# templeblock/audioSignalProcess

Hardware: AMD Instinct MI355X
Metric: audio frames/sec (10 ms @16 kHz) Wiener NS (higher is better)
Workload: dtype f32

## Files before the change

audiosignalprocess_amd/csrc/ns_kernels1.hip:

```cpp
#include <hip/hip_runtime.h>

#include "handoff.h"
#include "ns_device.h"
#include "ns_layout.h"
#include "ns_pair_fft.h"

namespace {
using namespace asphandoff;
using namespace aspns_dev;
using namespace aspns_pair;

__device__ __forceinline__ unsigned long long ns_cu_tag() {
  const unsigned hw = __builtin_amdgcn_s_getreg((7 << 11) | (8 << 6) | 4);
  const unsigned xcc = __builtin_amdgcn_s_getreg((3 << 11) | (0 << 6) | 20);
  return (unsigned long long)((xcc << 8) | hw);
}

constexpr int NS3 = 3;

__device__ __forceinline__ int ns_cold(int x) {
  asm volatile("" : "+v"(x));
  return x;
}
template <typename P>
__device__ __forceinline__ const P* ns_cold(const P* p) {
  asm volatile("" : "+s"(p));
  return p;
}

struct NsFlowArgs {
  HandoffArgs hand;
  unsigned want;
  int slot0;
  int ring;
  unsigned per;
  unsigned steps;
  unsigned walk;
};

template <bool IO16>
__device__ __forceinline__ float4 load_frame4(const float* in, size_t idx) {
  if constexpr (IO16) {
    const short4 a = *reinterpret_cast<const short4*>(reinterpret_cast<const short*>(in) + idx);
    return make_float4((float)a.x, (float)a.y, (float)a.z, (float)a.w);
  } else {
    return *reinterpret_cast<const float4*>(in + idx);
  }
}

constexpr int kImgDwords = aspns::kOffVec + aspns::V_HOT_COUNT * aspns::kVecStride;
constexpr int kImgVec4 = kImgDwords / (64 * 4);
static_assert(kImgDwords == 1792 && kImgDwords % (64 * 4) == 0, "the image is copied as whole 16-byte pieces per lane");
typedef __attribute__((address_space(3))) float lds_f32;
typedef __attribute__((address_space(3))) f32x2v lds_f32x2;
typedef __attribute__((address_space(3))) f32x4v lds_f32x4;

template <bool FLOW>
struct StateAcc {
  float* st;
  __amdgpu_buffer_rsrc_t rs;
  lds_f32* img;
  __device__ __forceinline__ StateAcc(float* p, float* image) : st(p), img((lds_f32*)image) {
    if constexpr (FLOW) rs = __builtin_amdgcn_make_buffer_rsrc(p, 0, aspns::kStreamDwords * 4, 0x00020000);
  }
  __device__ __forceinline__ float ld1(int uni, int vec) const {
    if constexpr (FLOW) return uni < kImgDwords ? img[uni + vec] : sc1_load1(rs, vec * 4, uni * 4);
    else return st[uni + vec];
  }
  __device__ __forceinline__ float2 ld2(int uni, int vec) const {
    if constexpr (FLOW) {
      if (uni >= kImgDwords) return sc1_load2(rs, vec * 4, uni * 4);
      const f32x2v v = *reinterpret_cast<const lds_f32x2*>(img + uni + vec);
      return make_float2(v.x, v.y);
    } else {
      return *reinterpret_cast<const float2*>(st + uni + vec);
    }
  }
  __device__ __forceinline__ float4 ld4(int uni, int vec) const {
    if constexpr (FLOW) {
      if (uni >= kImgDwords) return sc1_load4(rs, vec * 4, uni * 4);
      const f32x4v v = *reinterpret_cast<const lds_f32x4*>(img + uni + vec);
      return make_float4(v.x, v.y, v.z, v.w);
    } else {
      return *reinterpret_cast<const float4*>(st + uni + vec);
    }
  }
  __device__ __forceinline__ void st1(int uni, int vec, float v) const {
    if constexpr (FLOW) {
      if (uni < kImgDwords) img[uni + vec] = v;
      else sc1_store1(rs, vec * 4, uni * 4, v);
    } else {
      st[uni + vec] = v;
    }
  }
  __device__ __forceinline__ void st2(int uni, int vec, float a, float b) const {
    if constexpr (FLOW) {
      if (uni < kImgDwords) *reinterpret_cast<lds_f32x2*>(img + uni + vec) = f32x2v{a, b};
      else sc1_store2(rs, vec * 4, uni * 4, a, b);
    } else {
      *reinterpret_cast<float2*>(st + uni + vec) = make_float2(a, b);
    }
  }
  __device__ __forceinline__ void st4(int uni, int vec, float4 x) const {
    if constexpr (FLOW) {
      if (uni < kImgDwords) *reinterpret_cast<lds_f32x4*>(img + uni + vec) = f32x4v{x.x, x.y, x.z, x.w};
      else sc1_store4(rs, vec * 4, uni * 4, x);
    } else {
      *reinterpret_cast<float4*>(st + uni + vec) = x;
    }
  }
  __device__ __forceinline__ void image_request(int lane, float4 (&v)[kImgVec4]) const {
#pragma unroll
    for (int i = 0; i < kImgVec4; ++i) v[i] = sc1_load4(rs, lane * 16, i * 1024);
  }
  __device__ __forceinline__ void image_fill(int lane, const float4 (&v)[kImgVec4]) const {
#pragma unroll
    for (int i = 0; i < kImgVec4; ++i)
      *reinterpret_cast<lds_f32x4*>(img + i * 256 + 4 * lane) = f32x4v{v[i].x, v[i].y, v[i].z, v[i].w};
  }
  __device__ __forceinline__ void image_write_back(int lane) const {
#pragma unroll
    for (int i = 0; i < kImgVec4; ++i) {
      const f32x4v v = *reinterpret_cast<const lds_f32x4*>(img + i * 256 + 4 * lane);
      sc1_store4(rs, lane * 16, i * 1024, make_float4(v.x, v.y, v.z, v.w));
    }
  }
};

template <bool IO16, bool FLOW>
__global__ __launch_bounds__(256, 4) void ns_frame1_kernel(float* __restrict__ state,
                                                           int32_t* __restrict__ hist_all,
                                                           const NsTables* __restrict__ T,
                                                           const float* __restrict__ in,
                                                           float* __restrict__ out,
                                                           int num_streams,
                                                           unsigned long long* __restrict__ stamps,
                                                           int stamp_mode, NsFlowArgs fa) {
#ifdef NS1_BUDGET
#define NS_STAMP(k)                                                                \
  __builtin_amdgcn_sched_barrier(0);                                               \
  asm volatile("; NS_PHASE " #k);                                                  \
  __builtin_amdgcn_sched_barrier(0);
#define NS_STEADY(x) __builtin_assume(x)
#else
  const int stamp_on = (stamps != nullptr && threadIdx.x < 64) ? (stamp_mode != 0 ? 1 : 2) : 0;
#define NS_STAMP(k)                                                                          \
  if (__builtin_amdgcn_readfirstlane(stamp_on) != 0 && threadIdx.x == 0) {                   \
    __builtin_amdgcn_sched_barrier(0);                                                       \
    if (stamp_on == 1) {                                                                     \
      if ((k) == 0 || (k) == 1 || (k) == 14 || (k) == 15)                                    \
        stamps[blockIdx.x * 4 + ((k) == 0 ? 0 : (k) == 1 ? 1 : (k) == 14 ? 2 : 3)] =        \
            __builtin_amdgcn_s_memrealtime() | ((k) == 0 ? ns_cu_tag() << 48 : 0ull);       \
    } else if (FLOW ? (blockIdx.x == gridDim.x / 2 && flow_j == fa.steps / 2)                \
                    : blockIdx.x == 0) {                                                     \
      stamps[k] = __builtin_amdgcn_s_memtime();                                              \
    }                                                                                        \
    __builtin_amdgcn_sched_barrier(0);                                                       \
  }
#define NS_STEADY(x)
#endif
  unsigned flow_j = 0, flow_end = 1, flow_slot = 0;
  if constexpr (FLOW) {
    flow_j = blockIdx.y * fa.walk;
    flow_end = flow_j + fa.walk < fa.steps ? flow_j + fa.walk : fa.steps;
    flow_slot = ((unsigned)fa.slot0 + flow_j) % (unsigned)fa.ring;
  } else {
    NS_STAMP(0)
  }
  __shared__ __align__(16) float2 lds[4][130];
  __shared__ __align__(16) float tabs[3 * 64 * 4 + 32 * 4 * 2];
  __shared__ __align__(16) float wins[kAnal];
  __shared__ __align__(16) double exp2s[64];
  __shared__ __align__(16) double2 logts[128];
  __shared__ __align__(16) float imgs[FLOW ? 4 : 1][FLOW ? kImgDwords : 4];
  const int tid = threadIdx.x;
  const float4* tab_src = tid < 192 ? reinterpret_cast<const float4*>(&T->tw[0][0][0]) + tid
                                    : reinterpret_cast<const float4*>(&T->spl[0][0][0]) + (tid - 192);
  const float4 tab_v = *tab_src;
  const float4 win_v = reinterpret_cast<const float4*>(T->window)[tid & 63];
  const double exp2_v = T->exp2_64[tid & 63];
  const double2 logt_v = reinterpret_cast<const double2*>(T->logtab)[tid & 127];
  const int lane = tid & 63;
  const int diagbits = T->diag[lane];
  const int wv = __builtin_amdgcn_readfirstlane(tid >> 6);
  float2* tile = lds[wv];
  const int lam = lane >> 1, h = lane & 1;
  const int g = lam >> 4, q = lam & 15;
  const int binA = q + 64 * g + 16 * h;
  const uint32_t gmask = g ? 0x80000000u : 0u;
  const int stream_raw = blockIdx.x * 4 + wv;
  bool wave_live = stream_raw < num_streams;
  const int stream = wave_live ? stream_raw : num_streams - 1;
  float* __restrict__ st = state + (size_t)stream * kStreamDwords;
  int32_t* __restrict__ hist = hist_all + (size_t)stream * kHistDwords;
  const StateAcc<FLOW> sa(st, FLOW ? imgs[wv] : nullptr);
  float* outj = out;

  float sv;
#define SC_I(k) __builtin_amdgcn_readlane(__float_as_int(sv), (k))
#define SC_F(k) __int_as_float(SC_I(k))
#define SC_SET_I(k, val) sv = writelane_bits<(k)>(sv, (int)(val))
#define SC_SET_F(k, val) sv = setlane_vgpr<(k)>(sv, (val))
  float4 s4;
  float2 carryA, carryB;
  float4 s4in = make_float4(0.f, 0.f, 0.f, 0.f);
  const size_t frame_uni = (size_t)stream * kBlockL;
  auto flow_load_in = [&](unsigned slot) __attribute__((always_inline)) {
    const int lane_c = ns_cold(lane);
    const unsigned frame_lane = 4u * (unsigned)((lane_c < 24 ? 24 : lane_c) - 24);
    const float* base = IO16 ? reinterpret_cast<const float*>(reinterpret_cast<const short*>(in + (size_t)slot * fa.per) + frame_uni)
                             : in + (size_t)slot * fa.per + frame_uni;
    s4in = load_frame4<IO16>(base, frame_lane);
  };
  auto flow_head = [&]() __attribute__((always_inline)) {
    NS_STAMP(0)
    outj = out + (size_t)flow_slot * fa.per;
    const int lane_c = ns_cold(lane);
    const float4 ha = sa.ld4(kOffAnaHist, 4 * (lane_c < 24 ? lane_c : 23));
    const bool hsel = lane_c < 24;
    s4.x = hsel ? ha.x : s4in.x;
    s4.y = hsel ? ha.y : s4in.y;
    s4.z = hsel ? ha.z : s4in.z;
    s4.w = hsel ? ha.w : s4in.w;
    const int q2_c = lane_c & 30;
    carryA = sa.ld2(kOffSynt, q2_c + 32 * (lane_c & 1));
    carryB = sa.ld2(kOffSynt, q2_c + 64);
  };
  [[maybe_unused]] float4 img_v[FLOW ? kImgVec4 : 1];
  if constexpr (FLOW) {
    flow_load_in(flow_slot);
    if (wave_live) wave_live = handoff_wait(fa.hand, fa.want + flow_j, stream, lane);
    if (wave_live) sa.image_request(lane, img_v);
  } else {
    sv = st[kOffScalars + lane];
    float* hbuf = st + kOffAnaHist;
    if (!IO16) {
      const float* src = lane < 24 ? hbuf + 4 * lane : in + (size_t)stream * kBlockL + 4 * (lane - 24);
      s4 = *reinterpret_cast<const float4*>(src);
    } else {
      const int lh = lane < 24 ? lane : 23, li = lane < 24 ? 24 : lane;
      const float4 ha = *reinterpret_cast<const float4*>(hbuf + 4 * lh);
      const short* in16 = reinterpret_cast<const short*>(in) + (size_t)stream * kBlockL + 4 * (li - 24);
      const short4 a = *reinterpret_cast<const short4*>(in16);
      const bool hsel = lane < 24;
      s4.x = hsel ? ha.x : (float)a.x;
      s4.y = hsel ? ha.y : (float)a.y;
      s4.z = hsel ? ha.z : (float)a.z;
      s4.w = hsel ? ha.w : (float)a.w;
    }
    carryA = *reinterpret_cast<const float2*>(st + kOffSynt + 2 * q + 32 * h);
    carryB = *reinterpret_cast<const float2*>(st + kOffSynt + 2 * q + 64);
  }

  reinterpret_cast<float4*>(tabs)[tid] = tab_v;
  if (tid < 64) exp2s[tid] = exp2_v;
  if (tid < 128) logts[tid] = logt_v;
  if (tid >= 192) reinterpret_cast<float4*>(wins)[tid - 192] = win_v;
  if constexpr (FLOW) {
    if (wave_live) sa.image_fill(lane, img_v);
  }
  __syncthreads();
  if (!wave_live) return;
  if constexpr (FLOW) {
    sv = sa.ld1(kOffScalars, lane);
    flow_head();
  }
  const float* tws = tabs;
  const float* spls = tabs + 3 * 64 * 4;
  const PairFftLane fl = pair_fft_lane(lane, diagbits);

#define LOADV(dst, f)                                                                          \
  {                                                                                            \
    const float2 v2_ = sa.ld2(kOffVec + (f)*kVecStride, 2 * lane);                             \
    dst[0] = v2_.x; dst[1] = v2_.y;                                                            \
  }
#define LOADT(dst, f) dst[2] = SC_F(S_TAIL0 + (f));
#define LOAD3(dst, f) LOADV(dst, f) LOADT(dst, f)
#define STORE3(f, srcv)                                                                        \
  {                                                                                            \
    sa.st2(kOffVec + (f)*kVecStride, 2 * lane, srcv[0], srcv[1]);                              \
    SC_SET_F(S_TAIL0 + (f), srcv[2]);                                                          \
  }
#define NS_NEXT_FRAME()                                                                        \
  if constexpr (FLOW) {                                                                        \
    flow_slot = flow_slot + 1u == (unsigned)fa.ring ? 0u : flow_slot + 1u;                     \
    if (flow_j + 1u < flow_end) flow_load_in(flow_slot);                                       \
  }
#define NS_STREAM_DONE()                                                                       \
  if constexpr (FLOW) {                                                                        \
    const bool walk_done_ = flow_j + 1u >= flow_end;                                           \
    if (walk_done_) {                                                                          \
      const int lane_w_ = ns_cold(lane);                                                       \
      sa.st1(kOffScalars, lane_w_, sv);                                                        \
      lds_sync1();                                                                             \
      sa.image_write_back(lane_w_);                                                            \
      handoff_drain();                                                                         \
    }                                                                                          \
    NS_STAMP(16)                                                                               \
    if (walk_done_) {                                                                          \
      if (lane == 0) handoff_publish(fa.hand.seq + stream, fa.want + flow_j);                  \
      return;                                                                                  \
    }                                                                                          \
    ++flow_j;                                                                                  \
    lds_sync1();                                                                               \
    flow_head();                                                                               \
    continue;                                                                                  \
  } else {                                                                                     \
    return;                                                                                    \
  }

  for (;;) {
    float LQ[3][NS3], DEN[3][NS3], quant[NS3];
    float smooth[NS3], noisePrev[NS3], magnPrevA[NS3], logLrt[NS3], avgPause[NS3];


    const float4 w4 = *reinterpret_cast<const float4*>(wins + 4 * lane);
    const float wx0 = w4.x * s4.x, wx1 = w4.y * s4.y, wx2 = w4.z * s4.z, wx3 = w4.w * s4.w;
    float epart = wx0 * wx0;
    epart += wx1 * wx1;
    epart += wx2 * wx2;
    epart += wx3 * wx3;
    const float energy1 = wave_sum_bcast(epart);

    {
      const int lane_c = ns_cold(lane);
      if (lane_c >= 40) sa.st4(kOffAnaHist, 4 * (lane_c - 40), s4);
    }

    NS_STEADY(energy1 != 0.0f);
    if (energy1 == 0.0f) {
      float* y = IO16 ? reinterpret_cast<float*>(reinterpret_cast<short*>(outj) + (size_t)stream * kBlockL)
                      : outj + (size_t)stream * kBlockL;
      NS_NEXT_FRAME()
      const int lane_c = ns_cold(lane);
      float2 o01 = make_float2(0.f, 0.f);
      if (lane_c < 48) o01 = sa.ld2(kOffSynt, 2 * lane_c);
      __builtin_amdgcn_fence(__ATOMIC_ACQ_REL, "wavefront");
      store2p<IO16>(y, 2 * lane_c, sat16p(o01.x), sat16p(o01.y));
      if (lane_c < 16) store2p<IO16>(y, 128 + 2 * lane_c, 0.f, 0.f);
      if (lane_c < 48) sa.st2(kOffSynt, 2 * lane_c, 0.f, 0.f);
      NS_STREAM_DONE()
    }

    LOADV(LQ[0], V_LQ0) LOADV(LQ[1], V_LQ1) LOADV(LQ[2], V_LQ2)
    LOADV(DEN[0], V_DEN0) LOADV(DEN[1], V_DEN1) LOADV(DEN[2], V_DEN2)
    LOADV(quant, V_QUANT)
    LOADT(quant, V_QUANT)
    NS_STAMP(1)
    *reinterpret_cast<float4*>(&tile[2 * lane]) = make_float4(wx0, wx1, wx2, wx3);
    lds_sync1();
    f32x2 er, ei;
    {
      f32x2 ea, eb;
      cft128_passes1(tile, tws, fl, lane, ea, eb);
      radix2_tail1(ea, eb, gmask, false, er, ei);
    }
    real_split1(tile, spls, lane, er, ei, false);

    NS_STAMP(2)
    LOADV(magnPrevA, V_MAGNPREV_A) LOADV(logLrt, V_LOGLRT) LOADV(avgPause, V_AVGPAUSE)
    LOADV(smooth, V_SMOOTH) LOADV(noisePrev, V_NOISEPREV)
    LOADT(magnPrevA, V_MAGNPREV_A) LOADT(logLrt, V_LOGLRT) LOADT(avgPause, V_AVGPAUSE)
    LOADT(smooth, V_SMOOTH) LOADT(noisePrev, V_NOISEPREV)

    float re[NS3], im[NS3], magn[NS3];
    re[0] = er.x;
    im[0] = ei.x;
    re[1] = er.y;
    im[1] = ei.y;
    re[2] = lane_bcast(ei.x, 0);
    im[2] = 0.f;
    if (lane == 0) im[0] = 0.f;
    {
      float m2[2] = {re[0] * re[0] + im[0] * im[0], re[1] * re[1] + im[1] * im[1]}, rt[2];
      fsqrt_n<2>(m2, rt);
      magn[0] = rt[0] + 1.f;
      magn[1] = rt[1] + 1.f;
    }
    if (lane == 0) magn[0] = fabsf(re[0]) + 1.f;
    magn[2] = fabsf(re[2]) + 1.f;

#define SUM3(v) (wave_sum_bcast(v[0] + v[1]) + v[2])

    int blockInd = SC_I(S_BLOCKIND);
    const float overdrive = SC_F(S_OVERDRIVE);
    const float denoiseBound = SC_F(S_DENOISEBOUND);
    float priorSpeechProb = SC_F(S_PRIORSPEECHPROB);
    const int gainmap = SC_I(S_GAINMAP);

    float noise[NS3], prevStsa[NS3];
    blockInd++;
    const int updateParsFlag = SC_I(S_MUP0);
    int updates = SC_I(S_UPDATES);
    int counter[3] = {SC_I(S_COUNTER0), SC_I(S_COUNTER1), SC_I(S_COUNTER2)};
    NS_STEADY(blockInd > NS_END_STARTUP_LONG + 1);
    NS_STEADY(updates >= NS_END_STARTUP_LONG);
    NS_STEADY(counter[0] < NS_END_STARTUP_LONG - 1 && counter[1] < NS_END_STARTUP_LONG - 1 && counter[2] < NS_END_STARTUP_LONG - 1);
    NS_STEADY(counter[0] >= 0 && counter[1] >= 0 && counter[2] >= 0);
    NS_STEADY(updateParsFlag >= 1);
    NS_STEADY(gainmap == 1);

    float lmagn[NS3];
    log_f32_via_tab_n<NS3>(magn, lmagn, logts);

    NS_STAMP(3)
    float signalEnergy, sumMagn, flatNum, avgPauseMean;
    {
      float p_se = (re[0] * re[0] + im[0] * im[0]) + (re[1] * re[1] + im[1] * im[1]);
      float p_sm = magn[0] + magn[1];
      float p_fl = lane == 0 ? lmagn[1] : lmagn[0] + lmagn[1];
      float p_ap = avgPause[0] + avgPause[1];
      wave_sums_bcast(p_se, p_sm, p_fl, p_ap);
      signalEnergy = p_se + (re[2] * re[2] + im[2] * im[2]);
      sumMagn = p_sm + magn[2];
      flatNum = p_fl + lmagn[2];
      avgPauseMean = p_ap + avgPause[2];
      signalEnergy = DIV129(signalEnergy);
    }

    NS_STAMP(4)
    if (updates < NS_END_STARTUP_LONG) updates++;
    bool quant_new = false;
    constexpr int kLqLane = S_TAIL0 + V_LQ0, kDenLane = S_TAIL0 + V_DEN0;
    static_assert(V_LQ1 == V_LQ0 + 1 && V_LQ2 == V_LQ0 + 2 && V_DEN1 == V_DEN0 + 1 && V_DEN2 == V_DEN0 + 2 &&
                  kDenLane == kLqLane + 3 && kLqLane / 16 == (kDenLane + 2) / 16,
                  "the tracker tails: three + three consecutive lanes of one DPP row");
    float lqT = sv, denT = dpp_move<0x103>(sv);
    float rcnt1v;
    {
      const int cntb = lanes3_bits<kLqLane>(counter[0], counter[1], counter[2]);
      const float cntv = (float)cntb, cnt1v = (float)(cntb + 1);
      rcnt1v = fdiv(1.f, cnt1v);
      tracker_step1(lqT, denT, lmagn[2], cntv, cnt1v, rcnt1v);
    }
#pragma unroll
    for (int s = 0; s < 3; ++s) {
      {
        const float cnt = (float)counter[s];
        const float cnt1 = (float)(counter[s] + 1);
        const float rcnt1 = lane_bcast(rcnt1v, kLqLane + s);
        f32x2 lq = {LQ[s][0], LQ[s][1]}, den = {DEN[s][0], DEN[s][1]};
        tracker_step2(lq, den, f32x2{lmagn[0], lmagn[1]}, cnt, cnt1, rcnt1);
        LQ[s][0] = lq.x; LQ[s][1] = lq.y;
        DEN[s][0] = den.x; DEN[s][1] = den.y;
      }
      if (counter[s] >= NS_END_STARTUP_LONG) {
        counter[s] = 0;
        if (updates >= NS_END_STARTUP_LONG) {
          LQ[s][2] = lane_bcast(lqT, kLqLane + s);
          exp_f32_via_f64_n<NS3>(LQ[s], quant, exp2s);
          quant_new = true;
        }
      }
      counter[s]++;
    }
    if (updates < NS_END_STARTUP_LONG) {
      LQ[2][2] = lane_bcast(lqT, kLqLane + 2);
      exp_f32_via_f64_n<NS3>(LQ[2], quant, exp2s);
      quant_new = true;
    }
#pragma unroll
    for (int k = 0; k < NS3; ++k) noise[k] = quant[k];
#pragma unroll
    for (int s = 0; s < 3; ++s) sa.st2(kOffVec + (V_LQ0 + s) * kVecStride, 2 * lane, LQ[s][0], LQ[s][1]);
#pragma unroll
    for (int s = 0; s < 3; ++s) sa.st2(kOffVec + (V_DEN0 + s) * kVecStride, 2 * lane, DEN[s][0], DEN[s][1]);
    sv = mergelanes_vgpr<(7ull << kLqLane)>(sv, lqT);
    sv = mergelanes_vgpr<(7ull << kDenLane)>(sv, dpp_move<0x113>(denT));
    if (quant_new) STORE3(V_QUANT, quant)

    NS_STAMP(5)
    float whiteNoiseLevel = SC_F(S_WHITE);
    float pinkNoiseNumerator = SC_F(S_PINKNUM);
    float pinkNoiseExp = SC_F(S_PINKEXP);
    float fd5 = SC_F(S_FD5);
    const bool startup = blockInd < NS_END_STARTUP_SHORT;
    if (startup) {
      const int binA_c = ns_cold(binA);
      const NsTables* Tc = ns_cold(T);
      float lm3[NS3], lilm[NS3];
#pragma unroll
      for (int k = 0; k < NS3; ++k) {
        const int bin = k < 2 ? binA_c + 32 * k : 128;
        const float li = Tc->logi[bin];
        lm3[k] = bin >= NS_START_BAND ? lmagn[k] : 0.f;
        lilm[k] = bin >= NS_START_BAND ? li * lmagn[k] : 0.f;
      }
      const float sum_log_magn = SUM3(lm3);
      const float sum_log_i_log_magn = SUM3(lilm);
      const float sum_log_i = Tc->sum_log_i, sum_log_i_square = Tc->sum_log_i_square;
      whiteNoiseLevel += DIV129(sumMagn) * overdrive;
      float tmpFloat1 = sum_log_i_square * ((float)(kBins - NS_START_BAND));
      tmpFloat1 -= (sum_log_i * sum_log_i);
      float tmpFloat2 = (sum_log_i_square * sum_log_magn - sum_log_i * sum_log_i_log_magn);
      float tmpFloat3 = tmpFloat2 / tmpFloat1;
      if (tmpFloat3 < 0.f) tmpFloat3 = 0.f;
      pinkNoiseNumerator += tmpFloat3;
      tmpFloat2 = (sum_log_i * sum_log_magn);
      tmpFloat2 -= ((float)(kBins - NS_START_BAND)) * sum_log_i_log_magn;
      tmpFloat3 = tmpFloat2 / tmpFloat1;
      if (tmpFloat3 < 0.f) tmpFloat3 = 0.f;
      if (tmpFloat3 > 1.f) tmpFloat3 = 1.f;
      pinkNoiseExp += tmpFloat3;
      float parametric_num = 0.f, parametric_exp = 0.f;
      if (pinkNoiseExp > 0.f) {
        parametric_num = (float)exp((double)(pinkNoiseNumerator / (float)(blockInd + 1)));
        parametric_num *= (float)(blockInd + 1);
        parametric_exp = pinkNoiseExp / (float)(blockInd + 1);
      }
      float pn[NS3];
#pragma unroll
      for (int k = 0; k < NS3; ++k) {
        const int bin = k < 2 ? binA_c + 32 * k : 128;
        if (pinkNoiseExp == 0.f) {
          pn[k] = whiteNoiseLevel;
        } else {
          const float use_band = (float)(bin < NS_START_BAND ? NS_START_BAND : bin);
          pn[k] = (float)((double)parametric_num / pow((double)use_band, (double)parametric_exp));
        }
        noise[k] *= (blockInd);
        const float t2 = pn[k] * (NS_END_STARTUP_SHORT - blockInd);
        noise[k] += (t2 / (float)(blockInd + 1));
        noise[k] /= NS_END_STARTUP_SHORT;
      }
      if constexpr (FLOW) {
        sa.st2(kOffVec + V_PARAMNOISE * kVecStride, 2 * ns_cold(lane), pn[0], pn[1]);
        SC_SET_F(S_TAIL0 + V_PARAMNOISE, pn[2]);
      } else {
        STORE3(V_PARAMNOISE, pn)
      }
    }
    if (blockInd < NS_END_STARTUP_LONG) {
      fd5 *= blockInd;
      fd5 += signalEnergy;
      fd5 /= (blockInd + 1);
    }

    NS_STAMP(6)
    float snrLocPost[NS3], snrLocPrior[NS3];
    {
      float dn1[NS3], dn2[NS3], q1[NS3], q2[NS3];
#pragma unroll
      for (int k = 0; k < NS3; ++k) {
        dn1[k] = noisePrev[k] + 0.0001f;
        dn2[k] = noise[k] + 0.0001f;
      }
      fdiv3(magnPrevA, dn1, q1);
      fdiv3(magn, dn2, q2);
#pragma unroll
      for (int k = 0; k < NS3; ++k) {
        const float previousEstimateStsa = q1[k] * smooth[k];
        prevStsa[k] = previousEstimateStsa;
        snrLocPost[k] = 0.f;
        if (magn[k] > noise[k]) snrLocPost[k] = q2[k] - 1.f;
        snrLocPrior[k] = NS_DD_PR_SNR * previousEstimateStsa + (1.f - NS_DD_PR_SNR) * snrLocPost[k];
      }
    }

    NS_STAMP(7)
    float fd0 = SC_F(S_FD0), fd4 = SC_F(S_FD4), fd6 = SC_F(S_FD6);
    float flatArg, flatDen;
    {
      float num = flatNum;
      float den = sumMagn - lane_bcast(magn[0], 0);
      den = DIV129(den);
      num = DIV129(num);
      flatArg = num;
      flatDen = den;
    }
    {
      float avgMagn = sumMagn;
      avgPauseMean = DIV129(avgPauseMean);
      avgMagn = DIV129(avgMagn);
      float cv[NS3], vp[NS3], vm[NS3];
#pragma unroll
      for (int k = 0; k < NS3; ++k) {
        const float dm = magn[k] - avgMagn, dp = avgPause[k] - avgPauseMean;
        cv[k] = dm * dp;
        vp[k] = dp * dp;
        vm[k] = dm * dm;
      }
      float covMagnPause = cv[0] + cv[1], varPause = vp[0] + vp[1], varMagn = vm[0] + vm[1];
      wave_sums_bcast(covMagnPause, varPause, varMagn);
      covMagnPause += cv[2];
      varPause += vp[2];
      varMagn += vm[2];
      covMagnPause = DIV129(covMagnPause);
      varPause = DIV129(varPause);
      varMagn = DIV129(varMagn);
      fd6 += signalEnergy;
      float avgDiffNormMagn = varMagn - fdiv(covMagnPause * covMagnPause, varPause + 0.0001f);
      avgDiffNormMagn = fdiv(avgDiffNormMagn, fd5 + 0.0001f);
      fd4 += NS_SPECT_DIFF_TAVG * (avgDiffNormMagn - fd4);
    }

    NS_STAMP(8)
    {
      float t1[NS3], lt1[NS3];
#pragma unroll
      for (int k = 0; k < NS3; ++k) t1[k] = 1.f + 2.f * snrLocPrior[k];
      log_f32_via_tab_n<NS3>(t1, lt1, logts);
      float tn[NS3], td3[NS3], t2v[NS3];
#pragma unroll
      for (int k = 0; k < NS3; ++k) {
        tn[k] = 2.f * snrLocPrior[k];
        td3[k] = t1[k] + 0.0001f;
      }
      fdiv3(tn, td3, t2v);
#pragma unroll
      for (int k = 0; k < NS3; ++k) {
        const float t2 = t2v[k];
        const float besselTmp = (snrLocPost[k] + 1.f) * t2;
        logLrt[k] += NS_LRT_TAVG * (besselTmp - lt1[k] - logLrt[k]);
      }
    }
    float logLrtTimeAvgKsum = SUM3(logLrt);
    logLrtTimeAvgKsum = DIV129(logLrtTimeAvgKsum);
    float ev[NS3];
    {
      float nl[NS3];
#pragma unroll
      for (int k = 0; k < NS3; ++k) nl[k] = -logLrt[k];
      nl[2] = lane == 0 ? flatArg : nl[2];
      exp_f32_via_f64_n<NS3>(nl, ev, exp2s);
      const float spectralTmp = fdiv(lane_bcast(ev[2], 0), flatDen);
      fd0 += NS_SPECT_FL_TAVG * (spectralTmp - fd0);
      ev[2] = lane_bcast(ev[2], 1);
    }

    NS_STAMP(9)
    float fd3 = SC_F(S_FD3);
    PriorModel pm;
    pm.p0 = SC_F(S_PMP0);
    pm.p1 = SC_F(S_PMP1);
    pm.p3 = SC_F(S_PMP3);
    pm.p4 = SC_F(S_PMP4);
    pm.p5 = SC_F(S_PMP5);
    pm.p6 = SC_F(S_PMP6);
    const float pmp2 = SC_F(S_PMP2);
    int mup0 = updateParsFlag, mup3 = SC_I(S_MUP3);
    const int mup1 = SC_I(S_MUP1);
    NS_STEADY(mup3 > 2);
    bool window_closed = false;
    if (updateParsFlag >= 1) {
      mup3--;
      if (mup3 > 0) {
        const int lane_c = ns_cold(lane);
        const float fv = lane_c == 0 ? fd3 : (lane_c == 1 ? fd0 : fd4);
        const float bw = lane_c == 1 ? 0.05f : 0.1f, rbw = lane_c == 1 ? 1.0f / 0.05f : 1.0f / 0.1f;
        const float lim = lane_c == 1 ? kHist * 0.05f : kHist * 0.1f;
        if (lane_c < 3 && (fv < lim) && (fv >= 0.0f))
          atomicAdd(&hist[lane_c * kHistStride + (int)div_by_uniform(fv, bw, rbw)], 1);
      }
      if (mup3 == 0) {
        if constexpr (FLOW) handoff_drain();
        pm = close_histogram_window<FLOW>(hist, lane, mup1, mup0 >= 1, pm);
        if constexpr (FLOW) handoff_drain();
        window_closed = true;
        mup3 = mup1;
        if (updateParsFlag == 1) {
          mup0 = 0;
        } else {
          fd6 = fd6 / ((float)mup1);
          fd5 = 0.5f * (fd6 + fd5);
          fd6 = 0.f;
        }
      }
    }
    fd3 = logLrtTimeAvgKsum;
    {
      const float widthPrior0 = NS_WIDTH_PR_MAP, widthPrior1 = 2.f * NS_WIDTH_PR_MAP,
                  widthPrior2 = 2.f * NS_WIDTH_PR_MAP;
      const int sgnMap = (int)pmp2;
      float widthPrior = widthPrior0;
      if (logLrtTimeAvgKsum < pm.p0) widthPrior = widthPrior1;
      const float arg0 = widthPrior * (logLrtTimeAvgKsum - pm.p0);
      widthPrior = widthPrior0;
      if (sgnMap == 1 && (fd0 > pm.p1)) widthPrior = widthPrior1;
      if (sgnMap == -1 && (fd0 < pm.p1)) widthPrior = widthPrior1;
      const float arg1 = (float)sgnMap * widthPrior * (pm.p1 - fd0);
      widthPrior = widthPrior0;
      if (fd4 < pm.p3) widthPrior = widthPrior2;
      const float arg2 = widthPrior * (fd4 - pm.p3);
      const float arg = lane == 0 ? arg0 : (lane == 1 ? arg1 : arg2);
      const float th = tanh_f32_via_f64(arg, exp2s);
      const float indicator0 = 0.5f * (lane_bcast(th, 0) + 1.f);
      const float indicator1 = 0.5f * (lane_bcast(th, 1) + 1.f);
      const float indicator2 = 0.5f * (lane_bcast(th, 2) + 1.f);
      const float indPrior = pm.p4 * indicator0 + pm.p5 * indicator1 + pm.p6 * indicator2;
      priorSpeechProb += NS_PRIOR_UPDATE * (indPrior - priorSpeechProb);
      if (priorSpeechProb > 1.f) priorSpeechProb = 1.f;
      if (priorSpeechProb < 0.01f) priorSpeechProb = 0.01f;
    }
    float probSpeech[NS3];
    {
      const float gainPrior = fdiv(1.f - priorSpeechProb, priorSpeechProb + 0.0001f);
      {
        float pd[NS3];
        const float ones[NS3] = {1.f, 1.f, 1.f};
#pragma unroll
        for (int k = 0; k < NS3; ++k) {
          float invLrt = ev[k];
          invLrt = (float)gainPrior * invLrt;
          pd[k] = 1.f + invLrt;
        }
        fdiv3(ones, pd, probSpeech);
      }
    }

    NS_STAMP(10)
    {
      const int srcA = q > 0 ? lane - 2 : (h ? 30 + 32 * g : 31);
      const int srcB = q > 0 ? lane - 2 : (h ? 30 + 32 * g : 31 + 32 * g);
      const bool a_from1 = q == 0 && h == 0;
      const bool b_from1 = q > 0 || h == 1;
      const float a0 = __shfl(probSpeech[0], srcA, 64), a1 = __shfl(probSpeech[1], srcA, 64);
      const float b0 = __shfl(probSpeech[0], srcB, 64), b1 = __shfl(probSpeech[1], srcB, 64);
      float prevProb[NS3];
      prevProb[0] = a_from1 ? a1 : a0;
      prevProb[1] = b_from1 ? b1 : b0;
      prevProb[2] = lane_bcast(probSpeech[1], 63);
      {
        const F3 np(noisePrev), mg(magn), ps(probSpeech), ap(avgPause);
        const F3 x = (1.f - ps) * mg + ps * np;
        const F3 uS = NS_SPEECH_UPDATE * np + (1.f - NS_SPEECH_UPDATE) * x;
        const F3 uN = NS_NOISE_UPDATE * np + (1.f - NS_NOISE_UPDATE) * x;
        B3 oldSpeech = gt3(F3(prevProb), F3(NS_PROB_RANGE));
        oldSpeech.v[0] = oldSpeech.v[0] && lane != 0;
        const F3 uOld = sel3(oldSpeech, uS, uN);
        const F3 uNew = sel3(gt3(ps, F3(NS_PROB_RANGE)), uS, uN);
        min3(uOld, uNew).store(noise);
        sel3(lt3(ps, F3(NS_PROB_RANGE)), ap + NS_GAMMA_PAUSE * (mg - ap), ap).store(avgPause);
      }
    }
    STORE3(V_LOGLRT, logLrt) STORE3(V_AVGPAUSE, avgPause)
    STORE3(V_MAGNPREV_A, magn)

    NS_STAMP(11)
    float initMagn[NS3], pnoise[NS3];
    if (startup) {
      if constexpr (FLOW) {
        handoff_drain();
        const int lane2_c = 2 * ns_cold(lane);
        const float2 im_ = sa.ld2(kOffVec + V_INITMAGN * kVecStride, lane2_c);
        const float2 pn_ = sa.ld2(kOffVec + V_PARAMNOISE * kVecStride, lane2_c);
        initMagn[0] = im_.x; initMagn[1] = im_.y;
        pnoise[0] = pn_.x; pnoise[1] = pn_.y;
        LOADT(initMagn, V_INITMAGN) LOADT(pnoise, V_PARAMNOISE)
#pragma unroll
        for (int k = 0; k < NS3; ++k) initMagn[k] += magn[k];
        sa.st2(kOffVec + V_INITMAGN * kVecStride, lane2_c, initMagn[0], initMagn[1]);
        SC_SET_F(S_TAIL0 + V_INITMAGN, initMagn[2]);
      } else {
        LOAD3(initMagn, V_INITMAGN)
        LOAD3(pnoise, V_PARAMNOISE)
#pragma unroll
        for (int k = 0; k < NS3; ++k) initMagn[k] += magn[k];
        STORE3(V_INITMAGN, initMagn)
      }
    }
    float gainv[NS3];
    float gq1[NS3], gq2[NS3], snrP[NS3];
    {
      float gd1[NS3], gd2[NS3];
#pragma unroll
      for (int k = 0; k < NS3; ++k) gd1[k] = noise[k] + 0.0001f;
      fdiv3(magn, gd1, gq1);
#pragma unroll
      for (int k = 0; k < NS3; ++k) {
        float currentEstimateStsa = 0.f;
        if (magn[k] > noise[k]) currentEstimateStsa = gq1[k] - 1.f;
        snrP[k] = NS_DD_PR_SNR * prevStsa[k] + (1.f - NS_DD_PR_SNR) * currentEstimateStsa;
        gd2[k] = overdrive + snrP[k];
      }
      fdiv3(snrP, gd2, gq2);
    }
#pragma unroll
    for (int k = 0; k < NS3; ++k) {
      float gg = fmin_raw(fmax_raw(gq2[k], denoiseBound), 1.f);
      if (startup) {
        float tmp = (initMagn[k] - overdrive * pnoise[k]);
        tmp /= (initMagn[k] + 0.0001f);
        if (tmp < denoiseBound) tmp = denoiseBound;
        if (tmp > 1.f) tmp = 1.f;
        gg *= (blockInd);
        tmp *= (NS_END_STARTUP_SHORT - blockInd);
        gg += tmp;
        gg /= (NS_END_STARTUP_SHORT);
      }
      gainv[k] = gg;
      re[k] *= gg;
      im[k] *= gg;
    }
    STORE3(V_SMOOTH, gainv)
    STORE3(V_NOISEPREV, noise)

    NS_STAMP(12)
    NS_NEXT_FRAME()
    er = f32x2{re[0], re[1]};
    ei = f32x2{im[0], im[1]};
    if (lane == 0) ei.x = re[2];
    real_split1(tile, spls, lane, er, ei, true);
    lds_sync1();
    {
      const int base = 64 * g + q + 16 * h;
      float* tf = reinterpret_cast<float*>(tile);
      tf[2 * base] = er.x;
      tf[2 * base + 1] = ei.x;
      tf[2 * base + 64] = er.y;
      tf[2 * base + 65] = ei.y;
    }
    lds_sync1();
    f32x2 tr, ti;
    {
      f32x2 ea, eb;
      cft128_passes1(tile, tws, fl, lane, ea, eb);
      radix2_tail1(ea, eb, gmask, true, tr, ti);
    }
    const float td0 = tr.x * (2.f / kAnal), td1 = ti.x * (2.f / kAnal);
    const float td2 = tr.y * (2.f / kAnal), td3s = ti.y * (2.f / kAnal);

    NS_STAMP(13)
    float factor = 1.f;
    if (gainmap == 1 && blockInd > NS_END_STARTUP_LONG) {
      float factor1 = 1.f, factor2 = 1.f;
      float e2 = td0 * td0;
      e2 += td1 * td1;
      e2 += td2 * td2;
      e2 += td3s * td3s;
      const float energy2 = wave_sum_bcast(e2);
      float gain = fsqrt(fdiv(energy2, energy1 + 1.f));
      if (gain > NS_B_LIM) {
        factor1 = 1.f + 1.3f * (gain - NS_B_LIM);
        if (gain * factor1 > 1.f) factor1 = fdiv(1.f, gain);
      }
      if (gain < NS_B_LIM) {
        if (gain <= denoiseBound) gain = denoiseBound;
        factor2 = 1.f - 0.3f * (NS_B_LIM - gain);
      }
      factor = priorSpeechProb * factor1 + (1.f - priorSpeechProb) * factor2;
    }

    {
      float* y = IO16 ? reinterpret_cast<float*>(reinterpret_cast<short*>(outj) + (size_t)stream * kBlockL)
                      : outj + (size_t)stream * kBlockL;
      __builtin_amdgcn_fence(__ATOMIC_ACQ_REL, "wavefront");
      const int nA = 2 * ns_cold(binA), nB = nA + 64;
      const float2 wA = *reinterpret_cast<const float2*>(wins + nA);
      const float2 wB = *reinterpret_cast<const float2*>(wins + nB);
      const float cA0 = g == 0 ? carryA.x : 0.f, cA1 = g == 0 ? carryA.y : 0.f;
      const float cB0 = (g == 0 && h == 0) ? carryB.x : 0.f, cB1 = (g == 0 && h == 0) ? carryB.y : 0.f;
      const float oA0 = cA0 + factor * (wA.x * td0), oA1 = cA1 + factor * (wA.y * td1);
      const float oB0 = cB0 + factor * (wB.x * td2), oB1 = cB1 + factor * (wB.y * td3s);
      if (nA >= 160) {
        sa.st2(kOffSynt, nA - 160, oA0, oA1);
      } else {
        store2p<IO16>(y, nA, sat16p(oA0), sat16p(oA1));
      }
      if (nB >= 160) {
        sa.st2(kOffSynt, nB - 160, oB0, oB1);
      } else {
        store2p<IO16>(y, nB, sat16p(oB0), sat16p(oB1));
      }
    }

    NS_STAMP(14)
    SC_SET_I(S_UPDATES, updates);
    SC_SET_I(S_COUNTER0, counter[0]);
    SC_SET_I(S_COUNTER1, counter[1]);
    SC_SET_I(S_COUNTER2, counter[2]);
    SC_SET_I(S_MUP0, mup0);
    SC_SET_I(S_MUP3, mup3);
    SC_SET_F(S_SIGNALENERGY, signalEnergy);
    SC_SET_F(S_SUMMAGN, sumMagn);
    if (startup) {
      SC_SET_F(S_WHITE, whiteNoiseLevel);
      SC_SET_F(S_PINKNUM, pinkNoiseNumerator);
      SC_SET_F(S_PINKEXP, pinkNoiseExp);
    }
    if (window_closed) {
      SC_SET_F(S_PMP0, pm.p0);
      SC_SET_F(S_PMP1, pm.p1);
      SC_SET_F(S_PMP3, pm.p3);
      SC_SET_F(S_PMP4, pm.p4);
      SC_SET_F(S_PMP5, pm.p5);
      SC_SET_F(S_PMP6, pm.p6);
    }
    SC_SET_F(S_FD0, fd0);
    SC_SET_F(S_FD3, fd3);
    SC_SET_F(S_FD4, fd4);
    SC_SET_F(S_FD5, fd5);
    SC_SET_F(S_FD6, fd6);
    SC_SET_I(S_BLOCKIND, blockInd);
    SC_SET_F(S_PRIORSPEECHPROB, priorSpeechProb);
    if constexpr (!FLOW) sa.st1(kOffScalars, lane, sv);
    NS_STAMP(15)
    NS_STREAM_DONE()
  }
#undef NS_STREAM_DONE
#undef NS_NEXT_FRAME
#undef NS_STAMP
#undef SC_I
#undef SC_F
#undef SC_SET_I
#undef SC_SET_F
#undef LOAD3
#undef LOADV
#undef LOADT
#undef STORE3
#undef SUM3
}

}

namespace aspns {

hipError_t launch_ns_frame1(bool io16, float* state, int32_t* hist, const NsTables* T,
                            const float* in, float* out, int num_streams, hipStream_t s,
                            unsigned long long* stamps, int stamp_mode) {
  const dim3 grid((num_streams + 3) / 4), block(256);
  const NsFlowArgs none = {{nullptr, nullptr}, 0u, 0, 1, 0u, 1u, 1u};
  if (io16)
    hipLaunchKernelGGL((ns_frame1_kernel<true, false>), grid, block, 0, s, state, hist, T, in, out,
                       num_streams, stamps, stamp_mode, none);
  else
    hipLaunchKernelGGL((ns_frame1_kernel<false, false>), grid, block, 0, s, state, hist, T, in, out,
                       num_streams, stamps, stamp_mode, none);
  return hipGetLastError();
}

hipError_t launch_ns_frame1_flow(bool io16, float* state, int32_t* hist, const NsTables* T,
                                 const float* in, float* out, int num_streams, hipStream_t s,
                                 unsigned* seq, unsigned* abort_w, unsigned want, int steps, int walk, int slot0,
                                 int ring, size_t per, unsigned long long* stamps) {
  walk = walk < 1 ? 1 : (walk > steps ? steps : walk);
  const int gx = ((num_streams + 3) / 4 + 7) / 8 * 8;
  const dim3 grid(gx, (steps + walk - 1) / walk), block(256);
  const NsFlowArgs fa = {{seq, abort_w}, want, slot0, ring, (unsigned)per, (unsigned)steps, (unsigned)walk};
  if (io16)
    hipLaunchKernelGGL((ns_frame1_kernel<true, true>), grid, block, 0, s, state, hist, T, in, out,
                       num_streams, stamps, 0, fa);
  else
    hipLaunchKernelGGL((ns_frame1_kernel<false, true>), grid, block, 0, s, state, hist, T, in, out,
                       num_streams, stamps, 0, fa);
  return hipGetLastError();
}

}
```

Measured before the change: 441.6 million.

## Batch scalar prior and gain computation across waves via LDS mailbox server

In the FLOW path, each wave posts its per-frame scalar inputs (feature statistics and energy for the gain) into a mailbox in its LDS tile. A single rotating 'server' wave then computes the prior-speech-probability update (tanh, divisions) and the gain-compensation factor for all four streams at once, using 4-lane groups, and writes the results back. The goal is to stop every wave from running the serial scalar divisions and transcendentals separately. In exchange it adds two workgroup barriers per stage and ties the waves together in lockstep, which can cost more than the scalar work it saves.

```diff
diff --git a/audiosignalprocess_amd/csrc/ns_kernels1.hip b/audiosignalprocess_amd/csrc/ns_kernels1.hip
--- a/audiosignalprocess_amd/csrc/ns_kernels1.hip
+++ b/audiosignalprocess_amd/csrc/ns_kernels1.hip
@@ -126,6 +126,36 @@
     }
   }
 };
+
+constexpr int kTileDwords = 2 * 130;
+constexpr int kMbPriorIn = 64, kMbPriorOut = 76, kMbGainIn = 84, kMbGainOut = 92;
+static_assert(aspns::S_COUNT <= 64 && kMbGainOut < kTileDwords, "the mailbox fits the tile");
+
+__device__ __forceinline__ void ns_wg_barrier() { asm volatile("s_waitcnt lgkmcnt(0)\n\ts_barrier" ::: "memory"); }
+
+__device__ __forceinline__ int ns_pick_server(int live, int r) {
+  const int m = ((live | (live << 4)) >> r) & 15;
+  return (r + __builtin_ctz(m)) & 3;
+}
+
+__device__ __forceinline__ float ns_gain_factor(float energy1, float energy2, float priorSpeechProb,
+                                                float denoiseBound) {
+  float factor1 = 1.f, factor2 = 1.f;
+  float gain = fsqrt(fdiv(energy2, energy1 + 1.f));
+  if (gain > NS_B_LIM) {
+    factor1 = 1.f + 1.3f * (gain - NS_B_LIM);
+    if (gain * factor1 > 1.f) factor1 = fdiv(1.f, gain);
+  }
+  if (gain < NS_B_LIM) {
+    if (gain <= denoiseBound) gain = denoiseBound;
+    factor2 = 1.f - 0.3f * (NS_B_LIM - gain);
+  }
+  return priorSpeechProb * factor1 + (1.f - priorSpeechProb) * factor2;
+}
+
+#ifndef NS1_SHARE
+#define NS1_SHARE 3
+#endif
 
 template <bool IO16, bool FLOW>
 __global__ __launch_bounds__(256, 4) void ns_frame1_kernel(float* __restrict__ state,
@@ -173,6 +203,8 @@
   __shared__ __align__(16) double exp2s[64];
   __shared__ __align__(16) double2 logts[128];
   __shared__ __align__(16) float imgs[FLOW ? 4 : 1][FLOW ? kImgDwords : 4];
+  __shared__ __align__(16) int live_w[4];
+  constexpr bool kShareGain = FLOW && (NS1_SHARE & 1) != 0, kSharePrior = FLOW && (NS1_SHARE & 2) != 0;
   const int tid = threadIdx.x;
   const float4* tab_src = tid < 192 ? reinterpret_cast<const float4*>(&T->tw[0][0][0]) + tid
                                     : reinterpret_cast<const float4*>(&T->spl[0][0][0]) + (tid - 192);
@@ -258,16 +290,99 @@
   if (tid >= 192) reinterpret_cast<float4*>(wins)[tid - 192] = win_v;
   if constexpr (FLOW) {
     if (wave_live) sa.image_fill(lane, img_v);
+    if (lane == 0) live_w[wv] = wave_live ? 1 : 0;
   }
   __syncthreads();
   if (!wave_live) return;
+  [[maybe_unused]] int live_mask = 0;
   if constexpr (FLOW) {
     sv = sa.ld1(kOffScalars, lane);
     flow_head();
+    const int4 lw = *reinterpret_cast<const int4*>(live_w);
+    live_mask = __builtin_amdgcn_readfirstlane(lw.x | (lw.y << 1) | (lw.z << 2) | (lw.w << 3));
   }
   const float* tws = tabs;
   const float* spls = tabs + 3 * 64 * 4;
   const PairFftLane fl = pair_fft_lane(lane, diagbits);
+
+  struct PriorOut { float fd0, fd3, fd4, fd6, prior, gainPrior; };
+  [[maybe_unused]] auto share_prior = [&](bool valid, float sumLrt, float flatDenRaw, float evFlat, float sigEnergy,
+                                          float cov, float varP, float varM, float fd5v)
+                                          __attribute__((always_inline)) -> PriorOut {
+    const int lane_c = ns_cold(lane);
+    lds_f32* mb = (lds_f32*)reinterpret_cast<float*>(tile);
+    if (valid) mb[lane_c] = sv;
+    if (lane_c == 0) {
+      *reinterpret_cast<lds_f32x4*>(mb + kMbPriorIn) = f32x4v{sumLrt, flatDenRaw, evFlat, sigEnergy};
+      *reinterpret_cast<lds_f32x4*>(mb + kMbPriorIn + 4) = f32x4v{cov, varP, varM, fd5v};
+      mb[kMbPriorIn + 8] = valid ? 1.f : 0.f;
+    }
+    ns_wg_barrier();
+    if (ns_pick_server(live_mask, (int)(flow_j & 3u)) == wv) {
+      lds_f32* mk = (lds_f32*)reinterpret_cast<float*>(&lds[0][0]) + ((lane_c >> 2) & 3) * kTileDwords;
+      const int sub = lane_c & 3;
+      const f32x4v i0 = *reinterpret_cast<const lds_f32x4*>(mk + kMbPriorIn);
+      const f32x4v i1 = *reinterpret_cast<const lds_f32x4*>(mk + kMbPriorIn + 4);
+      const bool asked = mk[kMbPriorIn + 8] != 0.f;
+      float fd0 = mk[S_FD0], fd4 = mk[S_FD4], fd6 = mk[S_FD6], prior = mk[S_PRIORSPEECHPROB];
+      const float p0 = mk[S_PMP0], p1 = mk[S_PMP1], pmp2 = mk[S_PMP2], p3 = mk[S_PMP3];
+      const float p4 = mk[S_PMP4], p5 = mk[S_PMP5], p6 = mk[S_PMP6];
+      const float flatDen = DIV129(i0.y);
+      const float spectralTmp = fdiv(i0.z, flatDen);
+      fd0 += NS_SPECT_FL_TAVG * (spectralTmp - fd0);
+      const float covMagnPause = DIV129(i1.x), varPause = DIV129(i1.y), varMagn = DIV129(i1.z);
+      fd6 += i0.w;
+      float avgDiffNormMagn = varMagn - fdiv(covMagnPause * covMagnPause, varPause + 0.0001f);
+      avgDiffNormMagn = fdiv(avgDiffNormMagn, i1.w + 0.0001f);
+      fd4 += NS_SPECT_DIFF_TAVG * (avgDiffNormMagn - fd4);
+      const float logLrtTimeAvgKsum = DIV129(i0.x);
+      const float widthPrior0 = NS_WIDTH_PR_MAP, widthPrior1 = 2.f * NS_WIDTH_PR_MAP,
+                  widthPrior2 = 2.f * NS_WIDTH_PR_MAP;
+      const int sgnMap = (int)pmp2;
+      float widthPrior = widthPrior0;
+      if (logLrtTimeAvgKsum < p0) widthPrior = widthPrior1;
+      const float arg0 = widthPrior * (logLrtTimeAvgKsum - p0);
+      widthPrior = widthPrior0;
+      if (sgnMap == 1 && (fd0 > p1)) widthPrior = widthPrior1;
+      if (sgnMap == -1 && (fd0 < p1)) widthPrior = widthPrior1;
+      const float arg1 = (float)sgnMap * widthPrior * (p1 - fd0);
+      widthPrior = widthPrior0;
+      if (fd4 < p3) widthPrior = widthPrior2;
+      const float arg2 = widthPrior * (fd4 - p3);
+      const float arg = asked ? (sub == 0 ? arg0 : (sub == 1 ? arg1 : arg2)) : 0.f;
+      const float th = tanh_f32_via_f64(arg, exp2s);
+      const float indicator0 = 0.5f * (dpp_move<0x00>(th) + 1.f);
+      const float indicator1 = 0.5f * (dpp_move<0x55>(th) + 1.f);
+      const float indicator2 = 0.5f * (dpp_move<0xAA>(th) + 1.f);
+      const float indPrior = p4 * indicator0 + p5 * indicator1 + p6 * indicator2;
+      prior += NS_PRIOR_UPDATE * (indPrior - prior);
+      if (prior > 1.f) prior = 1.f;
+      if (prior < 0.01f) prior = 0.01f;
+      const float gainPrior = fdiv(1.f - prior, prior + 0.0001f);
+      if ((lane_c & 0x33) == 0) {
+        *reinterpret_cast<lds_f32x4*>(mk + kMbPriorOut) = f32x4v{fd0, logLrtTimeAvgKsum, fd4, fd6};
+        *reinterpret_cast<lds_f32x2*>(mk + kMbPriorOut + 4) = f32x2v{prior, gainPrior};
+      }
+    }
+    ns_wg_barrier();
+    const f32x4v o0 = *reinterpret_cast<const lds_f32x4*>(mb + kMbPriorOut);
+    const f32x2v o1 = *reinterpret_cast<const lds_f32x2*>(mb + kMbPriorOut + 4);
+    return PriorOut{o0.x, o0.y, o0.z, o0.w, o1.x, o1.y};
+  };
+  [[maybe_unused]] auto share_gain = [&](float e1, float e2, float psp, float db) __attribute__((always_inline)) -> float {
+    const int lane_c = ns_cold(lane);
+    lds_f32* mb = (lds_f32*)reinterpret_cast<float*>(tile);
+    if (lane_c == 0) *reinterpret_cast<lds_f32x4*>(mb + kMbGainIn) = f32x4v{e1, e2, psp, db};
+    ns_wg_barrier();
+    if (ns_pick_server(live_mask, (int)((flow_j + 2u) & 3u)) == wv) {
+      lds_f32* mk = (lds_f32*)reinterpret_cast<float*>(&lds[0][0]) + ((lane_c >> 2) & 3) * kTileDwords;
+      const f32x4v a = *reinterpret_cast<const lds_f32x4*>(mk + kMbGainIn);
+      const float f = ns_gain_factor(a.x, a.y, a.z, a.w);
+      if ((lane_c & 0x33) == 0) mk[kMbGainOut] = f;
+    }
+    ns_wg_barrier();
+    return mb[kMbGainOut];
+  };
 
 #define LOADV(dst, f)                                                                          \
   {                                                                                            \
@@ -339,6 +454,8 @@
       store2p<IO16>(y, 2 * lane_c, sat16p(o01.x), sat16p(o01.y));
       if (lane_c < 16) store2p<IO16>(y, 128 + 2 * lane_c, 0.f, 0.f);
       if (lane_c < 48) sa.st2(kOffSynt, 2 * lane_c, 0.f, 0.f);
+      if constexpr (kSharePrior) (void)share_prior(false, 0.f, 0.f, 0.f, 0.f, 0.f, 0.f, 0.f, 0.f);
+      if constexpr (kShareGain) (void)share_gain(0.f, 0.f, 0.f, 0.f);
       NS_STREAM_DONE()
     }
 
@@ -563,11 +680,12 @@
     {
       float num = flatNum;
       float den = sumMagn - lane_bcast(magn[0], 0);
-      den = DIV129(den);
+      if constexpr (!kSharePrior) den = DIV129(den);
       num = DIV129(num);
       flatArg = num;
       flatDen = den;
     }
+    [[maybe_unused]] float shCov = 0.f, shVarP = 0.f, shVarM = 0.f, shEvFlat = 0.f;
     {
       float avgMagn = sumMagn;
       avgPauseMean = DIV129(avgPauseMean);
@@ -585,13 +703,19 @@
       covMagnPause += cv[2];
       varPause += vp[2];
       varMagn += vm[2];
-      covMagnPause = DIV129(covMagnPause);
-      varPause = DIV129(varPause);
-      varMagn = DIV129(varMagn);
-      fd6 += signalEnergy;
-      float avgDiffNormMagn = varMagn - fdiv(covMagnPause * covMagnPause, varPause + 0.0001f);
-      avgDiffNormMagn = fdiv(avgDiffNormMagn, fd5 + 0.0001f);
-      fd4 += NS_SPECT_DIFF_TAVG * (avgDiffNormMagn - fd4);
+      if constexpr (kSharePrior) {
+        shCov = covMagnPause;
+        shVarP = varPause;
+        shVarM = varMagn;
+      } else {
+        covMagnPause = DIV129(covMagnPause);
+        varPause = DIV129(varPause);
+        varMagn = DIV129(varMagn);
+        fd6 += signalEnergy;
+        float avgDiffNormMagn = varMagn - fdiv(covMagnPause * covMagnPause, varPause + 0.0001f);
+        avgDiffNormMagn = fdiv(avgDiffNormMagn, fd5 + 0.0001f);
+        fd4 += NS_SPECT_DIFF_TAVG * (avgDiffNormMagn - fd4);
+      }
     }
 
     NS_STAMP(8)
@@ -615,7 +739,7 @@
       }
     }
     float logLrtTimeAvgKsum = SUM3(logLrt);
-    logLrtTimeAvgKsum = DIV129(logLrtTimeAvgKsum);
+    if constexpr (!kSharePrior) logLrtTimeAvgKsum = DIV129(logLrtTimeAvgKsum);
     float ev[NS3];
     {
       float nl[NS3];
@@ -623,8 +747,12 @@
       for (int k = 0; k < NS3; ++k) nl[k] = -logLrt[k];
       nl[2] = lane == 0 ? flatArg : nl[2];
       exp_f32_via_f64_n<NS3>(nl, ev, exp2s);
-      const float spectralTmp = fdiv(lane_bcast(ev[2], 0), flatDen);
-      fd0 += NS_SPECT_FL_TAVG * (spectralTmp - fd0);
+      if constexpr (kSharePrior) {
+        shEvFlat = lane_bcast(ev[2], 0);
+      } else {
+        const float spectralTmp = fdiv(lane_bcast(ev[2], 0), flatDen);
+        fd0 += NS_SPECT_FL_TAVG * (spectralTmp - fd0);
+      }
       ev[2] = lane_bcast(ev[2], 1);
     }
 
@@ -642,9 +770,32 @@
     const int mup1 = SC_I(S_MUP1);
     NS_STEADY(mup3 > 2);
     bool window_closed = false;
-    if (updateParsFlag >= 1) {
-      mup3--;
-      if (mup3 > 0) {
+    float gainPrior;
+    if constexpr (kSharePrior) {
+      bool hist_inc = false;
+      if (updateParsFlag >= 1) {
+        mup3--;
+        hist_inc = mup3 > 0;
+        if (mup3 == 0) {
+          handoff_drain();
+          pm = close_histogram_window<FLOW>(hist, lane, mup1, mup0 >= 1, pm);
+          handoff_drain();
+          window_closed = true;
+          mup3 = mup1;
+          if (updateParsFlag == 1) mup0 = 0;
+          SC_SET_F(S_PMP0, pm.p0);
+          SC_SET_F(S_PMP1, pm.p1);
+          SC_SET_F(S_PMP3, pm.p3);
+          SC_SET_F(S_PMP4, pm.p4);
+          SC_SET_F(S_PMP5, pm.p5);
+          SC_SET_F(S_PMP6, pm.p6);
+        }
+      }
+      const PriorOut po = share_prior(true, logLrtTimeAvgKsum, flatDen, shEvFlat, signalEnergy, shCov, shVarP, shVarM, fd5);
+      fd0 = po.fd0;
+      fd4 = po.fd4;
+      fd6 = po.fd6;
+      if (hist_inc) {
         const int lane_c = ns_cold(lane);
         const float fv = lane_c == 0 ? fd3 : (lane_c == 1 ? fd0 : fd4);
         const float bw = lane_c == 1 ? 0.05f : 0.1f, rbw = lane_c == 1 ? 1.0f / 0.05f : 1.0f / 0.1f;
@@ -652,49 +803,69 @@
         if (lane_c < 3 && (fv < lim) && (fv >= 0.0f))
           atomicAdd(&hist[lane_c * kHistStride + (int)div_by_uniform(fv, bw, rbw)], 1);
       }
-      if (mup3 == 0) {
-        if constexpr (FLOW) handoff_drain();
-        pm = close_histogram_window<FLOW>(hist, lane, mup1, mup0 >= 1, pm);
-        if constexpr (FLOW) handoff_drain();
-        window_closed = true;
-        mup3 = mup1;
-        if (updateParsFlag == 1) {
-          mup0 = 0;
-        } else {
-          fd6 = fd6 / ((float)mup1);
-          fd5 = 0.5f * (fd6 + fd5);
-          fd6 = 0.f;
+      if (window_closed && updateParsFlag != 1) {
+        fd6 = fd6 / ((float)mup1);
+        fd5 = 0.5f * (fd6 + fd5);
+        fd6 = 0.f;
+      }
+      fd3 = po.fd3;
+      priorSpeechProb = po.prior;
+      gainPrior = po.gainPrior;
+    } else {
+      if (updateParsFlag >= 1) {
+        mup3--;
+        if (mup3 > 0) {
+          const int lane_c = ns_cold(lane);
+          const float fv = lane_c == 0 ? fd3 : (lane_c == 1 ? fd0 : fd4);
+          const float bw = lane_c == 1 ? 0.05f : 0.1f, rbw = lane_c == 1 ? 1.0f / 0.05f : 1.0f / 0.1f;
+          const float lim = lane_c == 1 ? kHist * 0.05f : kHist * 0.1f;
+          if (lane_c < 3 && (fv < lim) && (fv >= 0.0f))
+            atomicAdd(&hist[lane_c * kHistStride + (int)div_by_uniform(fv, bw, rbw)], 1);
         }
-      }
-    }
-    fd3 = logLrtTimeAvgKsum;
-    {
-      const float widthPrior0 = NS_WIDTH_PR_MAP, widthPrior1 = 2.f * NS_WIDTH_PR_MAP,
-                  widthPrior2 = 2.f * NS_WIDTH_PR_MAP;
-      const int sgnMap = (int)pmp2;
-      float widthPrior = widthPrior0;
-      if (logLrtTimeAvgKsum < pm.p0) widthPrior = widthPrior1;
-      const float arg0 = widthPrior * (logLrtTimeAvgKsum - pm.p0);
-      widthPrior = widthPrior0;
-      if (sgnMap == 1 && (fd0 > pm.p1)) widthPrior = widthPrior1;
-      if (sgnMap == -1 && (fd0 < pm.p1)) widthPrior = widthPrior1;
-      const float arg1 = (float)sgnMap * widthPrior * (pm.p1 - fd0);
-      widthPrior = widthPrior0;
-      if (fd4 < pm.p3) widthPrior = widthPrior2;
-      const float arg2 = widthPrior * (fd4 - pm.p3);
-      const float arg = lane == 0 ? arg0 : (lane == 1 ? arg1 : arg2);
-      const float th = tanh_f32_via_f64(arg, exp2s);
-      const float indicator0 = 0.5f * (lane_bcast(th, 0) + 1.f);
-      const float indicator1 = 0.5f * (lane_bcast(th, 1) + 1.f);
-      const float indicator2 = 0.5f * (lane_bcast(th, 2) + 1.f);
-      const float indPrior = pm.p4 * indicator0 + pm.p5 * indicator1 + pm.p6 * indicator2;
-      priorSpeechProb += NS_PRIOR_UPDATE * (indPrior - priorSpeechProb);
-      if (priorSpeechProb > 1.f) priorSpeechProb = 1.f;
-      if (priorSpeechProb < 0.01f) priorSpeechProb = 0.01f;
+        if (mup3 == 0) {
+          if constexpr (FLOW) handoff_drain();
+          pm = close_histogram_window<FLOW>(hist, lane, mup1, mup0 >= 1, pm);
+          if constexpr (FLOW) handoff_drain();
+          window_closed = true;
+          mup3 = mup1;
+          if (updateParsFlag == 1) {
+            mup0 = 0;
+          } else {
+            fd6 = fd6 / ((float)mup1);
+            fd5 = 0.5f * (fd6 + fd5);
+            fd6 = 0.f;
+          }
+        }
+      }
+      fd3 = logLrtTimeAvgKsum;
+      {
+        const float widthPrior0 = NS_WIDTH_PR_MAP, widthPrior1 = 2.f * NS_WIDTH_PR_MAP,
+                    widthPrior2 = 2.f * NS_WIDTH_PR_MAP;
+        const int sgnMap = (int)pmp2;
+        float widthPrior = widthPrior0;
+        if (logLrtTimeAvgKsum < pm.p0) widthPrior = widthPrior1;
+        const float arg0 = widthPrior * (logLrtTimeAvgKsum - pm.p0);
+        widthPrior = widthPrior0;
+        if (sgnMap == 1 && (fd0 > pm.p1)) widthPrior = widthPrior1;
+        if (sgnMap == -1 && (fd0 < pm.p1)) widthPrior = widthPrior1;
+        const float arg1 = (float)sgnMap * widthPrior * (pm.p1 - fd0);
+        widthPrior = widthPrior0;
+        if (fd4 < pm.p3) widthPrior = widthPrior2;
+        const float arg2 = widthPrior * (fd4 - pm.p3);
+        const float arg = lane == 0 ? arg0 : (lane == 1 ? arg1 : arg2);
+        const float th = tanh_f32_via_f64(arg, exp2s);
+        const float indicator0 = 0.5f * (lane_bcast(th, 0) + 1.f);
+        const float indicator1 = 0.5f * (lane_bcast(th, 1) + 1.f);
+        const float indicator2 = 0.5f * (lane_bcast(th, 2) + 1.f);
+        const float indPrior = pm.p4 * indicator0 + pm.p5 * indicator1 + pm.p6 * indicator2;
+        priorSpeechProb += NS_PRIOR_UPDATE * (indPrior - priorSpeechProb);
+        if (priorSpeechProb > 1.f) priorSpeechProb = 1.f;
+        if (priorSpeechProb < 0.01f) priorSpeechProb = 0.01f;
+      }
+      gainPrior = fdiv(1.f - priorSpeechProb, priorSpeechProb + 0.0001f);
     }
     float probSpeech[NS3];
     {
-      const float gainPrior = fdiv(1.f - priorSpeechProb, priorSpeechProb + 0.0001f);
       {
         float pd[NS3];
         const float ones[NS3] = {1.f, 1.f, 1.f};
@@ -822,23 +993,21 @@
 
     NS_STAMP(13)
     float factor = 1.f;
-    if (gainmap == 1 && blockInd > NS_END_STARTUP_LONG) {
-      float factor1 = 1.f, factor2 = 1.f;
-      float e2 = td0 * td0;
-      e2 += td1 * td1;
-      e2 += td2 * td2;
-      e2 += td3s * td3s;
-      const float energy2 = wave_sum_bcast(e2);
-      float gain = fsqrt(fdiv(energy2, energy1 + 1.f));
-      if (gain > NS_B_LIM) {
-        factor1 = 1.f + 1.3f * (gain - NS_B_LIM);
-        if (gain * factor1 > 1.f) factor1 = fdiv(1.f, gain);
-      }
-      if (gain < NS_B_LIM) {
-        if (gain <= denoiseBound) gain = denoiseBound;
-        factor2 = 1.f - 0.3f * (NS_B_LIM - gain);
-      }
-      factor = priorSpeechProb * factor1 + (1.f - priorSpeechProb) * factor2;
+    {
+      const bool compensate = gainmap == 1 && blockInd > NS_END_STARTUP_LONG;
+      float energy2 = 0.f;
+      if (compensate) {
+        float e2 = td0 * td0;
+        e2 += td1 * td1;
+        e2 += td2 * td2;
+        e2 += td3s * td3s;
+        energy2 = wave_sum_bcast(e2);
+        if constexpr (!kShareGain) factor = ns_gain_factor(energy1, energy2, priorSpeechProb, denoiseBound);
+      }
+      if constexpr (kShareGain) {
+        const float f = share_gain(compensate ? energy1 : 0.f, energy2, priorSpeechProb, denoiseBound);
+        if (compensate) factor = f;
+      }
     }
 
     {
```

Measured after the change: 431.8 million. 2.2% lower.
